# AegisIK/DistMLIP

Hardware: NVIDIA B200
Metric: atoms/sec (energy+forces) CHGNet a-Si r_cut=5A (higher is better)
Workload: dtype f32

## Files before the change

### distmlip_b200/csrc/kernels_tc.cu

```cuda
#include "kernels.cuh"
#include "tc_common.cuh"

namespace b2m {

static int l2pf_level() {
  static const int v = [] {
    const char* e = getenv("B2M_L2_PREFETCH");
    return e ? atoi(e) : 1;
  }();
  return v;
}


__global__ void k_edge_basis(int64_t E, const float4* __restrict__ e_vec, RadialParams rp, float* __restrict__ be,
                             float* __restrict__ dbe) {
  const int64_t i = blockIdx.x * (int64_t)blockDim.x + threadIdx.x;
  if (i >= E * 3) return;
  const int64_t e = i / 3;
  const int part = (int)(i % 3);
  const float d = e_vec[e].w;
  float b[4] = {0.f, 0.f, 0.f, 0.f}, db[4] = {0.f, 0.f, 0.f, 0.f};
  for (int j = 0; j < 4; j++) {
    const int k = part * 4 + j;
    if (k < 9) rbf_env_both(d, rp.freq[k], rp, b[j], db[j]);
// ... 476 lines not shown
          const float4 g4 = *reinterpret_cast<const float4*>(gmrow + c);
          const float uu[4] = {u4.x, u4.y, u4.z, u4.w}, vv[4] = {v4.x, v4.y, v4.z, v4.w}, gg[4] = {g4.x, g4.y, g4.z, g4.w};
          float wab4[4], wabp4[4];
          radial_dot4(wabW, c, bek, wab4);
          if (br == 0) radial_dot4(wabW, c, dbek, wabp4);
#pragma unroll
          for (int j = 0; j < 4; j++) {
            const float wab = wab4[j];
            const float su = sigm_(uu[j]), oG = sigm_(vv[j]);
            const float oL = uu[j] * su;
            float g;
            if (br == 0) {
              g = gg[j] * oG * wab * (su * (1.f + uu[j] * (1.f - su)));
              gdpart = fmaf(gg[j] * oL * oG, wabp4[j], gdpart);
            } else {
              g = gg[j] * oL * wab * oG * (1.f - oG);
            }
            if (!valid) g = 0.f;
            const uint32_t h = tf32_hi_bits(g);
            hi[4 * i + j] = h;
            lo[4 * i + j] = __float_as_uint(g - __uint_as_float(h));
          }
        }
        tmem_st16(tlane + COL_H + c0 + ch * 16, hi);
        tmem_st16(tlane + COL_H + 64 + c0 + ch * 16, lo);
      }
      tc_wait_st();
      tc_fence_before();
      __syncthreads();
      if (tid == 0) {
        tc_fence_after();
        uint32_t acc = 0;
#pragma unroll
        for (int term = 0; term < 3; term++) {
          const uint32_t acol = term == 1 ? 64u : 0u;
          const uint32_t bsel = w2t_addr + (uint32_t)(br * 2 + (term == 2 ? 1 : 0)) * 4096u * 4u;
#pragma unroll
          for (int ks = 0; ks < 8; ks++) {
            umma_ts(tbase + COL_D + br * 64, tbase + COL_H + acol + ks * 8, umma_desc(bsel + ks * 2048u, 1024u, 128u),
                    kIdescN64, acc);
            acc = 1;
          }
        }
        umma_commit(&mbar[br + 1]);
      }
      mbar_wait_(&mbar[br + 1], phase);
      tc_fence_after();
#pragma unroll
      for (int ch = 0; ch < NCH; ch++) {
        uint32_t v[16];
        tmem_ld16(tlane + COL_D + br * 64 + c0 + ch * 16, v);
        tc_wait_ld();
#pragma unroll
        for (int i = 0; i < 16; i++) ds[ch * 16 + i] *= __uint_as_float(v[i]);
      }
      if (!viaQ) {
#pragma unroll
        for (int i = 0; i < CPT; i++) {
          const float4* Mj = reinterpret_cast<const float4*>(Mrow + (cb + i) * 12);
#pragma unroll
          for (int k4 = 0; k4 < 3; k4++) {
            const float4 m = Mj[k4];
            ffma2(gbeM[4 * k4], gbeM[4 * k4 + 1], ds[i], m.x, m.y);
            ffma2(gbeM[4 * k4 + 2], gbeM[4 * k4 + 3], ds[i], m.z, m.w);
          }
        }
      }
      if (need_gx) {
#pragma unroll 1
        for (int hp = 0; hp < 2; hp++) {
          if ((q >> 1) == hp) {
            const int rr = r - hp * 64;
#pragma unroll
            for (int i = 0; i < CPT; i++) stage[rr * 65 + c0 + i] = ds[i];
          }
          __syncthreads();
          {
            constexpr int RPP = 64 / (NTHR / 16);
            const int c4 = tid & 15, part = tid >> 4;
            const int col = br * 64 + c4 * 4;
            float s0 = 0.f, s1 = 0.f, s2 = 0.f, s3 = 0.f;
            int cur = -1;
            const int rbeg = part * RPP;
            for (int rr = rbeg; rr < rbeg + RPP; rr++) {
              const int row = hp * 64 + rr;
              const int k = s_dst[row];
              const float v0 = stage[rr * 65 + c4 * 4], v1 = stage[rr * 65 + c4 * 4 + 1], v2 = stage[rr * 65 + c4 * 4 + 2],
                          v3 = stage[rr * 65 + c4 * 4 + 3];
              if (k != cur) {
                if (cur >= 0) red_add_v4(&a.gC[(size_t)cur * D2 + col], s0, s1, s2, s3);
                cur = k;
                s0 = s1 = s2 = s3 = 0.f;
              }
              if (k >= 0) {
                s0 += v0, s1 += v1, s2 += v2, s3 += v3;
                red_add_v4(&a.gA[(size_t)s_src[row] * D2 + col], v0, v1, v2, v3);
                const int bnd = s_bond[row];
                if (useQ && bnd >= 0) *reinterpret_cast<float4*>(&a.gQ[(size_t)bnd * D2 + col]) = make_float4(v0, v1, v2, v3);
              }
            }
            if (cur >= 0) red_add_v4(&a.gC[(size_t)cur * D2 + col], s0, s1, s2, s3);
          }
          __syncthreads();
        }
      }
    }
    phase ^= 1;
    {
      float s = gdpart;
#pragma unroll
      for (int k = 0; k < 9; k++) s = fmaf(gbeM[k], dbek[k], s);
      stage[tid] = valid ? s : 0.f;
      tc_fence_before();
      __syncthreads();
      if (tid < nvalid) {
        float tot = 0.f;
#pragma unroll
        for (int pp = 0; pp < NP; pp++) tot += stage[pp * 128 + tid];
        a.gd[e0 + tid] += tot;
      }
      __syncthreads();
    }
  }
  tc_fence_before();
  __syncthreads();
  if (warp == 0) asm volatile("tcgen05.dealloc.cta_group::1.sync.aligned.b32 %0, %1;" ::"r"(tbase), "r"(256u));
}

void launch_atomconv_bwd_tc(cudaStream_t st, const AtomConvArgs& a, const AtomConvTcW& w, int num_sms) {
  if (a.E <= 0) return;
  static PerDeviceOnce attr;
  if (auto once_ = attr.first(); once_) {
    B2M_CK(cudaFuncSetAttribute(k_atomconv_bwd_tc<256>, cudaFuncAttributeMaxDynamicSharedMemorySize, (int)BwdTcSmem::bytes));
    B2M_CK(cudaFuncSetAttribute(k_atomconv_bwd_tc<512>, cudaFuncAttributeMaxDynamicSharedMemorySize, (int)BwdTcSmem::bytes));
  }
  const int64_t ntiles = (a.E + 127) / 128;
  const int grid = (int)std::min<int64_t>(ntiles, 2 * (int64_t)num_sms);
  static const int nthr = [] {
    const char* v = getenv("B2M_BWD_THREADS");
    return (v && atoi(v) == 512) ? 512 : 256;
  }();
  AtomConvTcW wl = w;
  wl.l2pf = l2pf_level() >= 1;
  if (nthr == 512)
    k_atomconv_bwd_tc<512><<<grid, 512, BwdTcSmem::bytes, st>>>(a, wl);
  else
    k_atomconv_bwd_tc<256><<<grid, 256, BwdTcSmem::bytes, st>>>(a, wl);
  B2M_CK(cudaGetLastError());
  g_launch_count++;
}

constexpr bool kFwdPrefetchDefault = true;
void launch_atomconv_fwd_tc(cudaStream_t st, const AtomConvArgs& a, const AtomConvTcW& w, int num_sms) {
  if (a.E <= 0) return;
  static PerDeviceOnce attr;
  if (auto once_ = attr.first(); once_) {
    B2M_CK(cudaFuncSetAttribute(k_atomconv_fwd_tc<256, false>, cudaFuncAttributeMaxDynamicSharedMemorySize, (int)FwdTcSmem::bytes));
    B2M_CK(cudaFuncSetAttribute(k_atomconv_fwd_tc<256, true>, cudaFuncAttributeMaxDynamicSharedMemorySize, (int)FwdTcSmem::bytes));
    B2M_CK(cudaFuncSetAttribute(k_atomconv_fwd_tc<512, false>, cudaFuncAttributeMaxDynamicSharedMemorySize, (int)FwdTcSmem::bytes));
  }
  const int64_t ntiles = (a.E + 127) / 128;
  const int grid = (int)std::min<int64_t>(ntiles, 2 * (int64_t)num_sms);
  static const int nthr = [] {
    const char* v = getenv("B2M_FWD_THREADS");
    return (v && atoi(v) == 512) ? 512 : 256;
  }();
  static const bool pf = [] {
    const char* v = getenv("B2M_FWD_PREFETCH");
    return v ? atoi(v) != 0 : kFwdPrefetchDefault;
  }();
  AtomConvTcW wl = w;
  wl.l2pf = l2pf_level() >= 1;
  if (nthr == 512)
    k_atomconv_fwd_tc<512, false><<<grid, 512, FwdTcSmem::bytes, st>>>(a, wl);
  else if (pf)
    k_atomconv_fwd_tc<256, true><<<grid, 256, FwdTcSmem::bytes, st>>>(a, wl);
  else
    k_atomconv_fwd_tc<256, false><<<grid, 256, FwdTcSmem::bytes, st>>>(a, wl);
  B2M_CK(cudaGetLastError());
  g_launch_count++;
}

}

namespace b2m {


struct LineTcSmem {
  static constexpr int kBar = 0;
  static constexpr int kWA = 64;
  static constexpr int kWB = kWA + 16384;
  static constexpr int kB2 = kWB + 16384;
  static constexpr int kGrp = kB2 + 128;
  static constexpr int kGrpSize = 64 * 65 + 2 * 3 * 128;
  static constexpr int kTotal = kGrp + 2 * kGrpSize;
  static constexpr size_t bytes = (size_t)kTotal * 4;
};

template <bool HIDDEN>
__global__ void __launch_bounds__(512, 1) k_line_fwd_tc(const LineArgs a, const LineTcW w) {
  extern __shared__ __align__(1024) float smem[];
  const int tid = threadIdx.x;
  const int g = tid >> 8, gt = tid & 255;
  const int warp = gt >> 5, lane = tid & 31;
  const int q = warp & 3, half = warp >> 2;
  const int r = q * 32 + lane, c0 = half * 32;
  uint64_t* mbar = reinterpret_cast<uint64_t*>(smem + LineTcSmem::kBar) + g * 6;
  uint32_t* tptr = reinterpret_cast<uint32_t*>(smem + LineTcSmem::kBar + 48);
  float* WAs = smem + LineTcSmem::kWA;
  float* WBs = smem + LineTcSmem::kWB;
  float* b2s = smem + LineTcSmem::kB2;
  float* stage = smem + LineTcSmem::kGrp + g * LineTcSmem::kGrpSize;
  int* s_a = reinterpret_cast<int*>(stage + 64 * 65);
  int* s_b = s_a + 128;
  int* s_c = s_b + 128;

  if ((tid >> 5) == 0) {
    asm volatile("tcgen05.alloc.cta_group::1.sync.aligned.shared::cta.b32 [%0], %1;" ::"r"(s_u32(tptr)), "r"(512u));
    asm volatile("tcgen05.relinquish_alloc_permit.cta_group::1.sync.aligned;");
  }
  if (gt == 0) {
    for (int i = 0; i < 6; i++) mbar_init_(&mbar[i], 1);
    asm volatile("fence.mbarrier_init.release.cluster;" ::: "memory");
  }
  if (gt < 128) {
    const int64_t e = (2 * (int64_t)blockIdx.x + g) * 128 + gt;
    const bool ok = e < a.A;
    s_a[gt] = ok ? a.a_in[e] : 0, s_b[gt] = ok ? a.a_out[e] : -1, s_c[gt] = ok ? a.a_ctr[e] : 0;
  }
  for (int i = tid; i < 4096; i += 512) reinterpret_cast<float4*>(WAs)[i] = reinterpret_cast<const float4*>(w.Wgcan)[i];
  if (HIDDEN)
    for (int i = tid; i < 4096; i += 512) reinterpret_cast<float4*>(WBs)[i] = reinterpret_cast<const float4*>(w.W2can)[i];
  if (tid < 128) b2s[tid] = (HIDDEN && a.b2) ? a.b2[tid] : 0.f;
  asm volatile("fence.proxy.async.shared::cta;" ::: "memory");
  tc_fence_before();
  __syncthreads();
  tc_fence_after();
  const uint32_t tbase = *tptr + (uint32_t)g * 256u;
  const uint32_t tlane = tbase + ((uint32_t)(q * 32) << 16);
  constexpr uint32_t COL_H = 0, COL_D = 128;
  const uint32_t wa_addr = s_u32(WAs), wb_addr = s_u32(WBs);
  uint32_t phase = 0;

  const int64_t ntiles = (a.A + 127) / 128;
  const int64_t tstride = 2 * (int64_t)gridDim.x;
  int* idxb = s_a;
  int buf = 0;
  for (int64_t t = 2 * (int64_t)blockIdx.x + g; t < ntiles; t += tstride, buf ^= 1) {
    const int64_t r0 = t * 128;
    const int nvalid = (int)min((int64_t)128, a.A - r0);
    const int64_t tn = t + tstride;
    s_a = idxb + buf * 384, s_b = s_a + 128, s_c = s_a + 256;
    int nia = 0, nib = -1, nic = 0;
    if (tn < ntiles && gt < 128 && tn * 128 + gt < a.A) nia = a.a_in[tn * 128 + gt], nib = a.a_out[tn * 128 + gt], nic = a.a_ctr[tn * 128 + gt];
    if (tn < ntiles) {
      asm volatile("prefetch.global.L2 [%0];" ::"l"(reinterpret_cast<const char*>(a.ang + tn * (128 * 64)) + gt * 128));
    }
    const bool valid = r < nvalid;
    const int ia = s_a[r], ib = s_b[r], ic = s_c[r];
    const float4* ang4 = reinterpret_cast<const float4*>(a.ang);
    float angv[32];
    {
#pragma unroll
      for (int ch = 0; ch < 2; ch++) {
        uint32_t hi[16], lo[16];
#pragma unroll
        for (int i = 0; i < 4; i++) {
          float4 x = ang4[tl4<16>(t, r, c0 + ch * 16 + i * 4)];
          if (!valid) x = make_float4(0.f, 0.f, 0.f, 0.f);
          const float xv[4] = {x.x, x.y, x.z, x.w};
#pragma unroll
          for (int j = 0; j < 4; j++) {
            angv[ch * 16 + 4 * i + j] = xv[j];
            const uint32_t h = tf32_hi_bits(xv[j]);
            hi[4 * i + j] = h;
            lo[4 * i + j] = __float_as_uint(xv[j] - __uint_as_float(h));
          }
        }
        tmem_st16(tlane + COL_H + c0 + ch * 16, hi);
        tmem_st16(tlane + COL_H + 64 + c0 + ch * 16, lo);
      }
    }
    tc_wait_st();
    tc_fence_before();
    gbar(g);
    if (gt == 0) {
      tc_fence_after();
      uint32_t acc = 0;
#pragma unroll
      for (int term = 0; term < 3; term++) {
        const uint32_t acol = term == 1 ? 64u : 0u;
        const uint32_t bsel = wa_addr + (term == 2 ? 8192u * 4u : 0u);
#pragma unroll
        for (int ks = 0; ks < 8; ks++) {
          umma_ts(tbase + COL_D, tbase + COL_H + acol + ks * 8, umma_desc(bsel + ks * 4096u, 2048u, 128u), kIdescN128, acc);
          acc = 1;
        }
      }
      umma_commit(&mbar[0]);
    }
    const float* Harow = a.Ha + (size_t)ia * D2;
    const float* Hbrow = a.Hb + (size_t)(valid ? ib : 0) * D2;
    const float* Xcrow = a.Xc + (size_t)ic * D2;
    if (HIDDEN) {
#pragma unroll 1
      for (int br = 0; br < 2; br++) {
        mbar_wait_(&mbar[br], phase);
        tc_fence_after();
        const int cb = br * 64 + c0;
#pragma unroll
        for (int ch = 0; ch < 2; ch++) {
          uint32_t v[16], hi[16], lo[16];
          tmem_ld16(tlane + COL_D + cb + ch * 16, v);
          tc_wait_ld();
          float dsv[16];
#pragma unroll
          for (int i = 0; i < 4; i++) {
            const float4 x = *reinterpret_cast<const float4*>(Harow + cb + ch * 16 + i * 4);
            const float4 y = *reinterpret_cast<const float4*>(Hbrow + cb + ch * 16 + i * 4);
            const float4 z = *reinterpret_cast<const float4*>(Xcrow + cb + ch * 16 + i * 4);
            const float p4[4] = {__uint_as_float(v[4 * i]) + x.x + y.x + z.x, __uint_as_float(v[4 * i + 1]) + x.y + y.y + z.y,
                                 __uint_as_float(v[4 * i + 2]) + x.z + y.z + z.z,
                                 __uint_as_float(v[4 * i + 3]) + x.w + y.w + z.w};
#pragma unroll
            for (int j = 0; j < 4; j++) {
              const float sg = sigm_(p4[j]);
              const float hval = valid ? p4[j] * sg : 0.f;
              dsv[4 * i + j] = sg * (1.f + p4[j] * (1.f - sg));
              const uint32_t h = tf32_hi_bits(hval);
              hi[4 * i + j] = h;
              lo[4 * i + j] = __float_as_uint(hval - __uint_as_float(h));
            }
          }
          if (a.ds_save != nullptr && valid) {
            float4* pd = reinterpret_cast<float4*>(a.ds_save);
#pragma unroll
            for (int i = 0; i < 4; i++)
              __stcs(&pd[tl4<32>(t, r, cb + ch * 16 + 4 * i)], make_float4(dsv[4 * i], dsv[4 * i + 1], dsv[4 * i + 2], dsv[4 * i + 3]));
          }
          tmem_st16(tlane + COL_H + c0 + ch * 16, hi);
          tmem_st16(tlane + COL_H + 64 + c0 + ch * 16, lo);
        }
        tc_wait_st();
        tc_fence_before();
        gbar(g);
        if (gt == 0) {
          tc_fence_after();
          uint32_t acc = 0;
#pragma unroll
          for (int term = 0; term < 3; term++) {
            const uint32_t acol = term == 1 ? 64u : 0u;
            const uint32_t bsel = wb_addr + (uint32_t)(br * 2 + (term == 2 ? 1 : 0)) * 4096u * 4u;
#pragma unroll
            for (int ks = 0; ks < 8; ks++) {
              umma_ts(tbase + COL_D + br * 64, tbase + COL_H + acol + ks * 8, umma_desc(bsel + ks * 2048u, 1024u, 128u),
                      kIdescN64, acc);
              acc = 1;
            }
          }
          umma_commit(&mbar[br + 1]);
        }
      }
      mbar_wait_(&mbar[2], phase);
      tc_fence_after();
    } else {
      mbar_wait_(&mbar[0], phase);
      tc_fence_after();
    }
    float mv[32];
#pragma unroll
    for (int ch = 0; ch < 2; ch++) {
      uint32_t u[16], v[16];
      tmem_ld16(tlane + COL_D + c0 + ch * 16, u);
      tmem_ld16(tlane + COL_D + 64 + c0 + ch * 16, v);
      tc_wait_ld();
      float uf[16], vf[16];
      if (HIDDEN) {
#pragma unroll
        for (int i = 0; i < 16; i++) {
          uf[i] = __uint_as_float(u[i]) + b2s[c0 + ch * 16 + i];
          vf[i] = __uint_as_float(v[i]) + b2s[64 + c0 + ch * 16 + i];
        }
      } else {
#pragma unroll
        for (int i = 0; i < 4; i++) {
          const int cL = c0 + ch * 16 + i * 4, cG = 64 + cL;
          const float4 x = *reinterpret_cast<const float4*>(Harow + cL);
          const float4 y = *reinterpret_cast<const float4*>(Hbrow + cL);
          const float4 z = *reinterpret_cast<const float4*>(Xcrow + cL);
          const float4 x2 = *reinterpret_cast<const float4*>(Harow + cG);
          const float4 y2 = *reinterpret_cast<const float4*>(Hbrow + cG);
          const float4 z2 = *reinterpret_cast<const float4*>(Xcrow + cG);
          uf[4 * i] = __uint_as_float(u[4 * i]) + x.x + y.x + z.x;
          uf[4 * i + 1] = __uint_as_float(u[4 * i + 1]) + x.y + y.y + z.y;
          uf[4 * i + 2] = __uint_as_float(u[4 * i + 2]) + x.z + y.z + z.z;
          uf[4 * i + 3] = __uint_as_float(u[4 * i + 3]) + x.w + y.w + z.w;
          vf[4 * i] = __uint_as_float(v[4 * i]) + x2.x + y2.x + z2.x;
          vf[4 * i + 1] = __uint_as_float(v[4 * i + 1]) + x2.y + y2.y + z2.y;
          vf[4 * i + 2] = __uint_as_float(v[4 * i + 2]) + x2.z + y2.z + z2.z;
          vf[4 * i + 3] = __uint_as_float(v[4 * i + 3]) + x2.w + y2.w + z2.w;
        }
      }
      if (a.uv_save != nullptr && valid) {
        float4* puv = reinterpret_cast<float4*>(a.uv_save);
#pragma unroll
        for (int i = 0; i < 4; i++) {
          __stcs(&puv[tl4<32>(t, r, c0 + ch * 16 + 4 * i)], make_float4(uf[4 * i], uf[4 * i + 1], uf[4 * i + 2], uf[4 * i + 3]));
          __stcs(&puv[tl4<32>(t, r, 64 + c0 + ch * 16 + 4 * i)], make_float4(vf[4 * i], vf[4 * i + 1], vf[4 * i + 2], vf[4 * i + 3]));
        }
      }
#pragma unroll
      for (int i = 0; i < 16; i++) mv[ch * 16 + i] = valid ? silu_(uf[i]) * sigm_(vf[i]) : 0.f;
    }
    phase ^= 1;
    tc_fence_before();
    if (HIDDEN) {
#pragma unroll 1
      for (int hp = 0; hp < 2; hp++) {
        if ((q >> 1) == hp) {
          const int rr = r - hp * 64;
#pragma unroll
          for (int i = 0; i < 32; i++) stage[rr * 65 + c0 + i] = mv[i];
        }
        gbar(g);
        {
          const int c = gt & 63, part = gt >> 6;
          float sum = 0.f;
          int cur = -1;
          const int rbeg = part * 16;
          for (int rr = rbeg; rr < rbeg + 16; rr++) {
            const int k = s_b[hp * 64 + rr];
            if (k != cur) {
              if (cur >= 0) atomicAdd(&a.aggB[(size_t)cur * D + c], sum);
              cur = k;
              sum = 0.f;
            }
            if (k >= 0) sum += stage[rr * 65 + c];
          }
          if (cur >= 0) atomicAdd(&a.aggB[(size_t)cur * D + c], sum);
        }
        if (hp == 1 && gt < 128) {
          int* nb_ = idxb + (buf ^ 1) * 384;
          nb_[gt] = nia, nb_[128 + gt] = nib, nb_[256 + gt] = nic;
        }
        gbar(g);
      }
    } else {
      if (valid) {
        float4* po = reinterpret_cast<float4*>(a.ang_out);
#pragma unroll
        for (int i = 0; i < 8; i++)
          po[tl4<16>(t, r, c0 + 4 * i)] = make_float4(angv[4 * i] + mv[4 * i], angv[4 * i + 1] + mv[4 * i + 1], angv[4 * i + 2] + mv[4 * i + 2],
                              angv[4 * i + 3] + mv[4 * i + 3]);
      }
      if (gt < 128) {
        int* nb_ = idxb + (buf ^ 1) * 384;
        nb_[gt] = nia, nb_[128 + gt] = nib, nb_[256 + gt] = nic;
      }
      gbar(g);
    }
  }
  tc_fence_before();
  __syncthreads();
  if ((tid >> 5) == 0) asm volatile("tcgen05.dealloc.cta_group::1.sync.aligned.b32 %0, %1;" ::"r"(*tptr), "r"(512u));
}

template <bool HIDDEN>
__global__ void __launch_bounds__(512, 1) k_line_bwd_tc(const LineArgs a, const LineTcW w) {
  extern __shared__ __align__(1024) float smem[];
  const int tid = threadIdx.x;
  const int g = tid >> 8, gt = tid & 255;
  const int warp = gt >> 5, lane = tid & 31;
  const int q = warp & 3, half = warp >> 2;
  const int r = q * 32 + lane, c0 = half * 32;
  uint64_t* mbar = reinterpret_cast<uint64_t*>(smem + LineTcSmem::kBar) + g * 6;
  uint32_t* tptr = reinterpret_cast<uint32_t*>(smem + LineTcSmem::kBar + 48);
  float* WAs = smem + LineTcSmem::kWA;
  float* WBs = smem + LineTcSmem::kWB;
  float* stage = smem + LineTcSmem::kGrp + g * LineTcSmem::kGrpSize;
  int* s_a = reinterpret_cast<int*>(stage + 64 * 65);
  int* s_b = s_a + 128;
  int* s_c = s_b + 128;

  if ((tid >> 5) == 0) {
    asm volatile("tcgen05.alloc.cta_group::1.sync.aligned.shared::cta.b32 [%0], %1;" ::"r"(s_u32(tptr)), "r"(512u));
    asm volatile("tcgen05.relinquish_alloc_permit.cta_group::1.sync.aligned;");
  }
  if (gt == 0) {
    for (int i = 0; i < 6; i++) mbar_init_(&mbar[i], 1);
    asm volatile("fence.mbarrier_init.release.cluster;" ::: "memory");
  }
  if (gt < 128) {
    const int64_t e = (2 * (int64_t)blockIdx.x + g) * 128 + gt;
    const bool ok = e < a.A;
    s_a[gt] = ok ? a.a_in[e] : -1, s_b[gt] = ok ? a.a_out[e] : -1, s_c[gt] = ok ? a.a_ctr[e] : -1;
  }
  for (int i = tid; i < 4096; i += 512) reinterpret_cast<float4*>(WAs)[i] = reinterpret_cast<const float4*>(w.WgTcan)[i];
  if (HIDDEN)
    for (int i = tid; i < 4096; i += 512) reinterpret_cast<float4*>(WBs)[i] = reinterpret_cast<const float4*>(w.W2Tcan)[i];
  asm volatile("fence.proxy.async.shared::cta;" ::: "memory");
  tc_fence_before();
  __syncthreads();
  tc_fence_after();
  const uint32_t tbase = *tptr + (uint32_t)g * 256u;
  const uint32_t tlane = tbase + ((uint32_t)(q * 32) << 16);
  constexpr uint32_t COL_H = 0, COL_D = 128, COL_G = 192;
  const uint32_t wa_addr = s_u32(WAs), wb_addr = s_u32(WBs);
  uint32_t phase = 0;

  const int64_t ntiles = (a.A + 127) / 128;
  const int64_t tstride = 2 * (int64_t)gridDim.x;
  int* idxb = s_a;
  int buf = 0;
  for (int64_t t = 2 * (int64_t)blockIdx.x + g; t < ntiles; t += tstride, buf ^= 1) {
    const int64_t r0 = t * 128;
    const int nvalid = (int)min((int64_t)128, a.A - r0);
    const int64_t tn = t + tstride;
    s_a = idxb + buf * 384, s_b = s_a + 128, s_c = s_a + 256;
    int nia = -1, nib = -1, nic = -1;
    if (tn < ntiles && gt < 128 && tn * 128 + gt < a.A) nia = a.a_in[tn * 128 + gt], nib = a.a_out[tn * 128 + gt], nic = a.a_ctr[tn * 128 + gt];
    if (tn < ntiles) {
      asm volatile("prefetch.global.L2 [%0];" ::"l"(reinterpret_cast<const char*>(a.gang + tn * (128 * 64)) + gt * 128));
      if (w.l2pf) {
        l2_prefetch(a.uv + tn * (128 * 128), 128 * 128 * 4, gt, 256);
        if (HIDDEN) l2_prefetch(a.ds + tn * (128 * 128), 128 * 128 * 4, gt, 256);
      }
    }
    const bool valid = r < nvalid;
    const int ib = s_b[r];
    const float4* uv4 = reinterpret_cast<const float4*>(a.uv);
    const float* gmrow = a.gaggB + (size_t)(valid && HIDDEN ? ib : 0) * D;
    const float4* gang4 = reinterpret_cast<const float4*>(a.gang);
#pragma unroll 1
    for (int br = 0; br < 2; br++) {
      float gp[32];
      const int cb = br * 64 + c0;
      if (br == 1) {
        mbar_wait_(&mbar[2], phase);
        tc_fence_after();
      }
#pragma unroll
      for (int ch = 0; ch < 2; ch++) {
        uint32_t hi[16], lo[16];
#pragma unroll
        for (int i = 0; i < 4; i++) {
          const int c = c0 + ch * 16 + i * 4;
          const float4 u4 = uv4[tl4<32>(t, r, c)];
          const float4 v4 = uv4[tl4<32>(t, r, 64 + c)];
          const float4 g4 = HIDDEN ? *reinterpret_cast<const float4*>(gmrow + c) : gang4[tl4<16>(t, r, c)];
          const float uu[4] = {u4.x, u4.y, u4.z, u4.w}, vv[4] = {v4.x, v4.y, v4.z, v4.w}, gg[4] = {g4.x, g4.y, g4.z, g4.w};
#pragma unroll
          for (int j = 0; j < 4; j++) {
            const float su = sigm_(uu[j]), oG = sigm_(vv[j]);
            float gval;
            if (br == 0)
              gval = gg[j] * oG * (su * (1.f + uu[j] * (1.f - su)));
            else
              gval = gg[j] * (uu[j] * su) * oG * (1.f - oG);
            if (!valid) gval = 0.f;
            gp[ch * 16 + 4 * i + j] = gval;
            const uint32_t h = tf32_hi_bits(gval);
            hi[4 * i + j] = h;
            lo[4 * i + j] = __float_as_uint(gval - __uint_as_float(h));
          }
        }
        if (HIDDEN) {
          tmem_st16(tlane + COL_H + c0 + ch * 16, hi);
          tmem_st16(tlane + COL_H + 64 + c0 + ch * 16, lo);
        }
      }
      if (HIDDEN) {
        tc_wait_st();
        tc_fence_before();
        gbar(g);
        if (gt == 0) {
          tc_fence_after();
          uint32_t acc = 0;
#pragma unroll
          for (int term = 0; term < 3; term++) {
            const uint32_t acol = term == 1 ? 64u : 0u;
            const uint32_t bsel = wb_addr + (uint32_t)(br * 2 + (term == 2 ? 1 : 0)) * 4096u * 4u;
#pragma unroll
            for (int ks = 0; ks < 8; ks++) {
              umma_ts(tbase + COL_D, tbase + COL_H + acol + ks * 8, umma_desc(bsel + ks * 2048u, 1024u, 128u), kIdescN64, acc);
              acc = 1;
            }
          }
          umma_commit(&mbar[br]);
        }
        const float4* ds4 = reinterpret_cast<const float4*>(a.ds);
        float4 dsr[8];
#pragma unroll
        for (int i = 0; i < 8; i++) dsr[i] = __ldcs(ds4 + tl4<32>(t, r, cb + i * 4));
        mbar_wait_(&mbar[br], phase);
        tc_fence_after();
#pragma unroll
        for (int ch = 0; ch < 2; ch++) {
          uint32_t v[16];
          tmem_ld16(tlane + COL_D + c0 + ch * 16, v);
          tc_wait_ld();
#pragma unroll
          for (int i = 0; i < 4; i++) {
            const float4 d4 = dsr[ch * 4 + i];
            gp[ch * 16 + 4 * i] = __uint_as_float(v[4 * i]) * d4.x;
            gp[ch * 16 + 4 * i + 1] = __uint_as_float(v[4 * i + 1]) * d4.y;
            gp[ch * 16 + 4 * i + 2] = __uint_as_float(v[4 * i + 2]) * d4.z;
            gp[ch * 16 + 4 * i + 3] = __uint_as_float(v[4 * i + 3]) * d4.w;
          }
        }
      }
#pragma unroll
      for (int ch = 0; ch < 2; ch++) {
        uint32_t hi[16], lo[16];
#pragma unroll
        for (int i = 0; i < 16; i++) {
          const float x = valid ? gp[ch * 16 + i] : 0.f;
          const uint32_t h = tf32_hi_bits(x);
          hi[i] = h;
          lo[i] = __float_as_uint(x - __uint_as_float(h));
        }
        tmem_st16(tlane + COL_H + c0 + ch * 16, hi);
        tmem_st16(tlane + COL_H + 64 + c0 + ch * 16, lo);
      }
      tc_wait_st();
      tc_fence_before();
      gbar(g);
      if (gt == 0) {
        tc_fence_after();
        uint32_t acc = br == 0 ? 0u : 1u;
#pragma unroll
        for (int term = 0; term < 3; term++) {
          const uint32_t acol = term == 1 ? 64u : 0u;
          const uint32_t bsel = wa_addr + (uint32_t)(br * 2 + (term == 2 ? 1 : 0)) * 4096u * 4u;
#pragma unroll
          for (int ks = 0; ks < 8; ks++) {
            umma_ts(tbase + COL_G, tbase + COL_H + acol + ks * 8, umma_desc(bsel + ks * 2048u, 1024u, 128u), kIdescN64, acc);
            acc = 1;
          }
        }
        umma_commit(&mbar[2 + br]);
      }
#pragma unroll 1
      for (int hp = 0; hp < 2; hp++) {
        if ((q >> 1) == hp) {
          const int rr = r - hp * 64;
#pragma unroll
          for (int i = 0; i < 32; i++) stage[rr * 65 + c0 + i] = gp[i];
        }
        gbar(g);
        {
          const int c4 = gt & 15, part = gt >> 4;
          const int col = br * 64 + c4 * 4;
          float sb0 = 0.f, sb1 = 0.f, sb2 = 0.f, sb3 = 0.f, sc0 = 0.f, sc1 = 0.f, sc2 = 0.f, sc3 = 0.f;
          int curb = -1, curc = -1;
          const int rbeg = part * 4;
          for (int rr = rbeg; rr < rbeg + 4; rr++) {
            const int rowi = hp * 64 + rr;
            const int kb = s_b[rowi], kc = s_c[rowi];
            const float v0 = stage[rr * 65 + c4 * 4], v1 = stage[rr * 65 + c4 * 4 + 1], v2 = stage[rr * 65 + c4 * 4 + 2],
                        v3 = stage[rr * 65 + c4 * 4 + 3];
            if (kb != curb) {
              if (curb >= 0) red_add_v4(&a.gHb[(size_t)curb * D2 + col], sb0, sb1, sb2, sb3);
              curb = kb;
              sb0 = sb1 = sb2 = sb3 = 0.f;
            }
            if (kc != curc) {
              if (curc >= 0) red_add_v4(&a.gXc[(size_t)curc * D2 + col], sc0, sc1, sc2, sc3);
              curc = kc;
              sc0 = sc1 = sc2 = sc3 = 0.f;
            }
            if (kb >= 0) {
              sb0 += v0, sb1 += v1, sb2 += v2, sb3 += v3;
              sc0 += v0, sc1 += v1, sc2 += v2, sc3 += v3;
              red_add_v4(&a.gHa[(size_t)s_a[rowi] * D2 + col], v0, v1, v2, v3);
            }
          }
          if (curb >= 0) red_add_v4(&a.gHb[(size_t)curb * D2 + col], sb0, sb1, sb2, sb3);
          if (curc >= 0) red_add_v4(&a.gXc[(size_t)curc * D2 + col], sc0, sc1, sc2, sc3);
        }
        gbar(g);
      }
    }
    {
      float4* pg = reinterpret_cast<float4*>(a.gang);
      float4 o[8];
#pragma unroll
      for (int i = 0; i < 8; i++) o[i] = valid ? pg[tl4<16>(t, r, c0 + 4 * i)] : make_float4(0.f, 0.f, 0.f, 0.f);
      mbar_wait_(&mbar[3], phase);
      tc_fence_after();
#pragma unroll
      for (int ch = 0; ch < 2; ch++) {
        uint32_t v[16];
        tmem_ld16(tlane + COL_G + c0 + ch * 16, v);
        tc_wait_ld();
        if (valid) {
#pragma unroll
          for (int i = 0; i < 4; i++) {
            float4 x = o[ch * 4 + i];
            x.x += __uint_as_float(v[4 * i]), x.y += __uint_as_float(v[4 * i + 1]);
            x.z += __uint_as_float(v[4 * i + 2]), x.w += __uint_as_float(v[4 * i + 3]);
            pg[tl4<16>(t, r, c0 + ch * 16 + 4 * i)] = x;
          }
        }
      }
    }
    phase ^= 1;
    if (gt < 128) {
      int* nb_ = idxb + (buf ^ 1) * 384;
      nb_[gt] = nia, nb_[128 + gt] = nib, nb_[256 + gt] = nic;
    }
    tc_fence_before();
    gbar(g);
  }
  tc_fence_before();
  __syncthreads();
  if ((tid >> 5) == 0) asm volatile("tcgen05.dealloc.cta_group::1.sync.aligned.b32 %0, %1;" ::"r"(*tptr), "r"(512u));
}

void launch_line_fwd_tc(cudaStream_t st, const LineArgs& a, const LineTcW& w, bool hidden, int num_sms) {
  if (a.A <= 0) return;
  static PerDeviceOnce attr;
  if (auto once_ = attr.first(); once_) {
    B2M_CK(cudaFuncSetAttribute(k_line_fwd_tc<true>, cudaFuncAttributeMaxDynamicSharedMemorySize, (int)LineTcSmem::bytes));
    B2M_CK(cudaFuncSetAttribute(k_line_fwd_tc<false>, cudaFuncAttributeMaxDynamicSharedMemorySize, (int)LineTcSmem::bytes));
  }
  const int64_t ntiles = (a.A + 127) / 128;
  const int grid = (int)std::min<int64_t>((ntiles + 1) / 2, (int64_t)num_sms);
  LineTcW wl = w;
  wl.l2pf = l2pf_level() >= 2;
  if (hidden)
    k_line_fwd_tc<true><<<grid, 512, LineTcSmem::bytes, st>>>(a, wl);
  else
    k_line_fwd_tc<false><<<grid, 512, LineTcSmem::bytes, st>>>(a, wl);
  B2M_CK(cudaGetLastError());
  g_launch_count++;
}
void launch_line_bwd_tc(cudaStream_t st, const LineArgs& a, const LineTcW& w, bool hidden, int num_sms) {
  if (a.A <= 0) return;
  static PerDeviceOnce attr;
  if (auto once_ = attr.first(); once_) {
    B2M_CK(cudaFuncSetAttribute(k_line_bwd_tc<true>, cudaFuncAttributeMaxDynamicSharedMemorySize, (int)LineTcSmem::bytes));
    B2M_CK(cudaFuncSetAttribute(k_line_bwd_tc<false>, cudaFuncAttributeMaxDynamicSharedMemorySize, (int)LineTcSmem::bytes));
// ... 385 lines not shown
```

### distmlip_b200/csrc/tc_common.cuh

```cuda
#pragma once
#include "kernels.cuh"

namespace b2m {

__device__ __forceinline__ float sigm_(float x) {
  float e, r;
  asm("ex2.approx.ftz.f32 %0, %1;" : "=f"(e) : "f"(x * -1.4426950408889634f));
  asm("rcp.approx.ftz.f32 %0, %1;" : "=f"(r) : "f"(1.f + e));
  return r;
}
__device__ __forceinline__ float silu_(float x) { return x * sigm_(x); }
__device__ __forceinline__ float dsilu_(float x) {
  const float sg = sigm_(x);
  return sg * (1.f + x * (1.f - sg));
}
__device__ __forceinline__ uint32_t s_u32(const void* p) { return (uint32_t)__cvta_generic_to_shared(p); }

__device__ __forceinline__ uint32_t tf32_hi_bits(float x) {
  uint32_t u;
  asm("cvt.rna.tf32.f32 %0, %1;" : "=r"(u) : "f"(x));
  return u;
}
__device__ __forceinline__ uint64_t umma_desc(uint32_t saddr, uint32_t lbo, uint32_t sbo) {
  return (uint64_t)((saddr & 0x3FFFF) >> 4) | ((uint64_t)(lbo >> 4) << 16) | ((uint64_t)(sbo >> 4) << 32) | (1ull << 46);
}
__device__ __forceinline__ void umma_ts(uint32_t d_tmem, uint32_t a_tmem, uint64_t bdesc, uint32_t idesc, uint32_t acc) {
  asm volatile(
      "{\n\t.reg .pred p;\n\tsetp.ne.b32 p, %4, 0;\n\t"
      "tcgen05.mma.cta_group::1.kind::tf32 [%0], [%1], %2, %3, p;\n\t}" ::"r"(d_tmem),
      "r"(a_tmem), "l"(bdesc), "r"(idesc), "r"(acc)
      : "memory");
}
__device__ __forceinline__ void umma_commit(uint64_t* bar) {
  asm volatile("tcgen05.commit.cta_group::1.mbarrier::arrive::one.shared::cluster.b64 [%0];" ::"r"(s_u32(bar)) : "memory");
}
__device__ __forceinline__ void tc_fence_before() { asm volatile("tcgen05.fence::before_thread_sync;" ::: "memory"); }
__device__ __forceinline__ void tc_fence_after() { asm volatile("tcgen05.fence::after_thread_sync;" ::: "memory"); }
__device__ __forceinline__ void tc_wait_st() { asm volatile("tcgen05.wait::st.sync.aligned;" ::: "memory"); }
__device__ __forceinline__ void tc_wait_ld() { asm volatile("tcgen05.wait::ld.sync.aligned;" ::: "memory"); }
__device__ __forceinline__ void tmem_st16(uint32_t addr, const uint32_t (&v)[16]) {
  asm volatile(
      "tcgen05.st.sync.aligned.32x32b.x16.b32 [%0], {%1, %2, %3, %4, %5, %6, %7, %8, %9, %10, %11, %12, %13, %14, %15, %16};" ::
          "r"(addr),
      "r"(v[0]), "r"(v[1]), "r"(v[2]), "r"(v[3]), "r"(v[4]), "r"(v[5]), "r"(v[6]), "r"(v[7]), "r"(v[8]), "r"(v[9]),
      "r"(v[10]), "r"(v[11]), "r"(v[12]), "r"(v[13]), "r"(v[14]), "r"(v[15])
      : "memory");
}
__device__ __forceinline__ void tmem_ld16(uint32_t addr, uint32_t (&v)[16]) {
  asm volatile(
      "tcgen05.ld.sync.aligned.32x32b.x16.b32 {%0, %1, %2, %3, %4, %5, %6, %7, %8, %9, %10, %11, %12, %13, %14, %15}, [%16];"
      : "=r"(v[0]), "=r"(v[1]), "=r"(v[2]), "=r"(v[3]), "=r"(v[4]), "=r"(v[5]), "=r"(v[6]), "=r"(v[7]), "=r"(v[8]),
        "=r"(v[9]), "=r"(v[10]), "=r"(v[11]), "=r"(v[12]), "=r"(v[13]), "=r"(v[14]), "=r"(v[15])
      : "r"(addr)
      : "memory");
}
__device__ __forceinline__ void mbar_init_(uint64_t* bar, uint32_t count) {
  asm volatile("mbarrier.init.shared::cta.b64 [%0], %1;" ::"r"(s_u32(bar)), "r"(count) : "memory");
}
__device__ __forceinline__ void mbar_wait_(uint64_t* bar, uint32_t parity) {
  uint32_t ok = 0;
  const uint32_t addr = s_u32(bar);
  do {
    asm volatile(
        "{\n\t.reg .pred p;\n\tmbarrier.try_wait.parity.shared::cta.b64 p, [%1], %2;\n\tselp.u32 %0, 1, 0, p;\n\t}"
        : "=r"(ok)
        : "r"(addr), "r"(parity)
        : "memory");
  } while (!ok);
}
__device__ __forceinline__ void gbar(int g) { asm volatile("bar.sync %0, 256;" ::"r"(g + 1) : "memory"); }
__device__ __forceinline__ float ipow_(float x, int n) {
  float r = 1.f;
  for (int i = 0; i < n; i++) r *= x;
  return r;
}
__device__ __forceinline__ float rbf_env_val(float d, float freq, const RadialParams& rp) {
  const float invd = 1.f / d;
  float s, c;
  sincosf(d * (freq / rp.rc), &s, &c);
  const float rbf = rp.norm * s * invd;
  const int p = rp.p;
  const float c1 = -(p + 1) * (p + 2) * 0.5f, c2 = (float)(p * (p + 2)), c3 = -p * (p + 1) * 0.5f;
  const float rho = rbf / rp.rc;
  const float r0 = ipow_(rho, p), r1 = r0 * rho, r2 = r1 * rho;
  const float env = 1.f + c1 * r0 + c2 * r1 + c3 * r2;
  return rbf <= rp.rc ? env * rbf : 0.f;
}

template <int NC4>
__device__ __forceinline__ size_t tl4(int64_t tile, int r, int c) {
  return ((size_t)(tile * NC4 + (c >> 2)) * 128 + r);
}

__device__ __forceinline__ void red_add_v4(float* addr, float a, float b, float c, float d) {
  asm volatile("red.global.add.v4.f32 [%0], {%1, %2, %3, %4};" ::"l"(addr), "f"(a), "f"(b), "f"(c), "f"(d) : "memory");
}

__device__ __forceinline__ void l2_prefetch(const void* base, int bytes, int tid, int nthr) {
  const char* p = reinterpret_cast<const char*>(base);
  for (int o = tid * 128; o < bytes; o += nthr * 128) asm volatile("prefetch.global.L2 [%0];" ::"l"(p + o));
}

__device__ __forceinline__ void ffma2(float& d0, float& d1, float a, float b0, float b1) {
  uint64_t A, B, C, D;
  asm("mov.b64 %0, {%1, %2};" : "=l"(A) : "f"(a), "f"(a));
  asm("mov.b64 %0, {%1, %2};" : "=l"(B) : "f"(b0), "f"(b1));
  asm("mov.b64 %0, {%1, %2};" : "=l"(C) : "f"(d0), "f"(d1));
  asm("fma.rn.f32x2 %0, %1, %2, %3;" : "=l"(D) : "l"(A), "l"(B), "l"(C));
  asm("mov.b64 {%0, %1}, %2;" : "=f"(d0), "=f"(d1) : "l"(D));
}
__device__ __forceinline__ void radial_dot16(const float* WT, int col0, const float (&b)[9], float (&w)[16]) {
#pragma unroll
  for (int i = 0; i < 16; i++) w[i] = 0.f;
#pragma unroll
  for (int k = 0; k < 9; k++) {
#pragma unroll
    for (int c4 = 0; c4 < 4; c4++) {
      const float4 x = *reinterpret_cast<const float4*>(WT + k * 64 + col0 + c4 * 4);
      ffma2(w[4 * c4], w[4 * c4 + 1], b[k], x.x, x.y);
      ffma2(w[4 * c4 + 2], w[4 * c4 + 3], b[k], x.z, x.w);
    }
  }
}

__device__ __forceinline__ void radial_dot4(const float* WT, int col0, const float (&b)[9], float (&w)[4]) {
  w[0] = w[1] = w[2] = w[3] = 0.f;
#pragma unroll
  for (int k = 0; k < 9; k++) {
    const float4 x = *reinterpret_cast<const float4*>(WT + k * 64 + col0);
    ffma2(w[0], w[1], b[k], x.x, x.y);
    ffma2(w[2], w[3], b[k], x.z, x.w);
  }
}

constexpr uint32_t kIdescN64 = (1u << 4) | (2u << 7) | (2u << 10) | (8u << 17) | (8u << 24);
constexpr uint32_t kIdescN128 = (1u << 4) | (2u << 7) | (2u << 10) | (16u << 17) | (8u << 24);

__device__ __forceinline__ void rbf_env_both(float d, float freq, const RadialParams& rp, float& be, float& dbe) {
  const float invd = 1.f / d;
  const float wq = freq / rp.rc;
  float s, c;
  sincosf(d * wq, &s, &c);
  const float rbf = rp.norm * s * invd;
  const float drbf = rp.norm * (wq * c * invd - s * invd * invd);
  const int p = rp.p;
  const float c1 = -(p + 1) * (p + 2) * 0.5f, c2 = (float)(p * (p + 2)), c3 = -p * (p + 1) * 0.5f;
  const float rho = rbf / rp.rc;
  const float rm1 = ipow_(rho, p - 1);
  const float r0 = rm1 * rho, r1 = r0 * rho, r2 = r1 * rho;
  const float env = 1.f + c1 * r0 + c2 * r1 + c3 * r2;
  const float denv = (c1 * p * rm1 + c2 * (p + 1) * r0 + c3 * (p + 2) * r1) / rp.rc;
  const bool ok = rbf <= rp.rc;
  be = ok ? env * rbf : 0.f;
  dbe = ok ? (env + rbf * denv) * drbf : 0.f;
}

__device__ __forceinline__ void mbar_expect_tx_(uint64_t* bar, uint32_t bytes) {
  asm volatile("mbarrier.arrive.expect_tx.shared::cta.b64 _, [%0], %1;" ::"r"(s_u32(bar)), "r"(bytes) : "memory");
}
__device__ __forceinline__ void bulk_g2s_(void* dst_smem, const void* src_gmem, uint32_t bytes, uint64_t* bar) {
  asm volatile("cp.async.bulk.shared::cluster.global.mbarrier::complete_tx::bytes [%0], [%1], %2, [%3];" ::"r"(
                   s_u32(dst_smem)),
               "l"(src_gmem), "r"(bytes), "r"(s_u32(bar))
               : "memory");
}


__device__ __forceinline__ void tmem_st8(uint32_t addr, const uint32_t (&v)[8]) {
  asm volatile("tcgen05.st.sync.aligned.32x32b.x8.b32 [%0], {%1, %2, %3, %4, %5, %6, %7, %8};" ::"r"(addr), "r"(v[0]),
               "r"(v[1]), "r"(v[2]), "r"(v[3]), "r"(v[4]), "r"(v[5]), "r"(v[6]), "r"(v[7])
               : "memory");
}
__device__ __forceinline__ void tmem_ld8(uint32_t addr, uint32_t (&v)[8]) {
  asm volatile("tcgen05.ld.sync.aligned.32x32b.x8.b32 {%0, %1, %2, %3, %4, %5, %6, %7}, [%8];"
               : "=r"(v[0]), "=r"(v[1]), "=r"(v[2]), "=r"(v[3]), "=r"(v[4]), "=r"(v[5]), "=r"(v[6]), "=r"(v[7])
               : "r"(addr)
               : "memory");
}
__device__ __forceinline__ void cp_async16_(void* dst_smem, const void* src_gmem) {
  asm volatile("cp.async.cg.shared.global [%0], [%1], 16;" ::"r"(s_u32(dst_smem)), "l"(src_gmem) : "memory");
}
__device__ __forceinline__ void cp_async_arrive_(uint64_t* bar) {
  asm volatile("cp.async.mbarrier.arrive.noinc.shared::cta.b64 [%0];" ::"r"(s_u32(bar)) : "memory");
}

__device__ __forceinline__ uint64_t pk2(float a, float b) {
  uint64_t r;
  asm("mov.b64 %0, {%1, %2};" : "=l"(r) : "f"(a), "f"(b));
  return r;
}
__device__ __forceinline__ void upk2(uint64_t v, float& a, float& b) { asm("mov.b64 {%0, %1}, %2;" : "=f"(a), "=f"(b) : "l"(v)); }
__device__ __forceinline__ uint64_t add2(uint64_t a, uint64_t b) {
  uint64_t r;
  asm("add.rn.f32x2 %0, %1, %2;" : "=l"(r) : "l"(a), "l"(b));
  return r;
}
__device__ __forceinline__ uint64_t sub2(uint64_t a, uint64_t b) {
  uint64_t r;
  asm("sub.rn.f32x2 %0, %1, %2;" : "=l"(r) : "l"(a), "l"(b));
  return r;
}
__device__ __forceinline__ uint64_t mul2(uint64_t a, uint64_t b) {
  uint64_t r;
  asm("mul.rn.f32x2 %0, %1, %2;" : "=l"(r) : "l"(a), "l"(b));
  return r;
}
__device__ __forceinline__ uint64_t fma2(uint64_t a, uint64_t b, uint64_t c) {
  uint64_t r;
  asm("fma.rn.f32x2 %0, %1, %2, %3;" : "=l"(r) : "l"(a), "l"(b), "l"(c));
  return r;
}
__device__ __forceinline__ float ex2_(float x) {
  float e;
  asm("ex2.approx.ftz.f32 %0, %1;" : "=f"(e) : "f"(x));
  return e;
}
__device__ __forceinline__ float rcp_(float x) {
  float r;
  asm("rcp.approx.ftz.f32 %0, %1;" : "=f"(r) : "f"(x));
  return r;
}
}
```

Before: 5.030 million.

## Prefetch next gather rows via bulk L2 prefetch, hoist row sums, vectorize scatter

Issues cp.async.bulk L2 prefetches for the next tile's Ha/Hb/Xc rows. The three-way gather sum is moved ahead of the mbarrier wait, so global loads overlap the tensor-core MMA. The segmented scatter-add now has each thread accumulate 4 columns over 4 rows and emit red.global.add.v4 instead of scalar atomicAdd, which cuts the number of atomic operations. The trade-offs are more register pressure from the early-loaded sums and shorter per-thread segments, which can mean more atomics when neighbours repeat. A profiling script is also added.

```diff
diff --git a/distmlip_b200/csrc/kernels_tc.cu b/distmlip_b200/csrc/kernels_tc.cu
--- a/distmlip_b200/csrc/kernels_tc.cu
+++ b/distmlip_b200/csrc/kernels_tc.cu
@@ -802,12 +802,23 @@
     const float* Harow = a.Ha + (size_t)ia * D2;
     const float* Hbrow = a.Hb + (size_t)(valid ? ib : 0) * D2;
     const float* Xcrow = a.Xc + (size_t)ic * D2;
+    auto prefetch_next_rows = [&] {
+      if (gt < 128 && nib >= 0) {
+        l2_prefetch_bulk(a.Ha + (size_t)nia * D2, D2 * 4);
+        l2_prefetch_bulk(a.Hb + (size_t)nib * D2, D2 * 4);
+        l2_prefetch_bulk(a.Xc + (size_t)nic * D2, D2 * 4);
+      }
+    };
+    float gsu[16];
     if (HIDDEN) {
+      prefetch_next_rows();
 #pragma unroll 1
       for (int br = 0; br < 2; br++) {
+        const int cb = br * 64 + c0;
+        float gs[32];
+        sum3_row(Harow + cb, Hbrow + cb, Xcrow + cb, gs);
         mbar_wait_(&mbar[br], phase);
         tc_fence_after();
-        const int cb = br * 64 + c0;
 #pragma unroll
         for (int ch = 0; ch < 2; ch++) {
           uint32_t v[16], hi[16], lo[16];
@@ -816,12 +827,9 @@
           float dsv[16];
 #pragma unroll
           for (int i = 0; i < 4; i++) {
-            const float4 x = *reinterpret_cast<const float4*>(Harow + cb + ch * 16 + i * 4);
-            const float4 y = *reinterpret_cast<const float4*>(Hbrow + cb + ch * 16 + i * 4);
-            const float4 z = *reinterpret_cast<const float4*>(Xcrow + cb + ch * 16 + i * 4);
-            const float p4[4] = {__uint_as_float(v[4 * i]) + x.x + y.x + z.x, __uint_as_float(v[4 * i + 1]) + x.y + y.y + z.y,
-                                 __uint_as_float(v[4 * i + 2]) + x.z + y.z + z.z,
-                                 __uint_as_float(v[4 * i + 3]) + x.w + y.w + z.w};
+            const float* s = gs + ch * 16 + i * 4;
+            const float p4[4] = {__uint_as_float(v[4 * i]) + s[0], __uint_as_float(v[4 * i + 1]) + s[1],
+                                 __uint_as_float(v[4 * i + 2]) + s[2], __uint_as_float(v[4 * i + 3]) + s[3]};
 #pragma unroll
             for (int j = 0; j < 4; j++) {
               const float sg = sigm_(p4[j]);
@@ -864,8 +872,10 @@
       mbar_wait_(&mbar[2], phase);
       tc_fence_after();
     } else {
+      sum3_row(Harow + c0, Hbrow + c0, Xcrow + c0, gsu);
       mbar_wait_(&mbar[0], phase);
       tc_fence_after();
+      prefetch_next_rows();
     }
     float mv[32];
 #pragma unroll
@@ -882,23 +892,18 @@
           vf[i] = __uint_as_float(v[i]) + b2s[64 + c0 + ch * 16 + i];
         }
       } else {
-#pragma unroll
-        for (int i = 0; i < 4; i++) {
-          const int cL = c0 + ch * 16 + i * 4, cG = 64 + cL;
-          const float4 x = *reinterpret_cast<const float4*>(Harow + cL);
-          const float4 y = *reinterpret_cast<const float4*>(Hbrow + cL);
-          const float4 z = *reinterpret_cast<const float4*>(Xcrow + cL);
-          const float4 x2 = *reinterpret_cast<const float4*>(Harow + cG);
-          const float4 y2 = *reinterpret_cast<const float4*>(Hbrow + cG);
-          const float4 z2 = *reinterpret_cast<const float4*>(Xcrow + cG);
-          uf[4 * i] = __uint_as_float(u[4 * i]) + x.x + y.x + z.x;
-          uf[4 * i + 1] = __uint_as_float(u[4 * i + 1]) + x.y + y.y + z.y;
-          uf[4 * i + 2] = __uint_as_float(u[4 * i + 2]) + x.z + y.z + z.z;
-          uf[4 * i + 3] = __uint_as_float(u[4 * i + 3]) + x.w + y.w + z.w;
-          vf[4 * i] = __uint_as_float(v[4 * i]) + x2.x + y2.x + z2.x;
-          vf[4 * i + 1] = __uint_as_float(v[4 * i + 1]) + x2.y + y2.y + z2.y;
-          vf[4 * i + 2] = __uint_as_float(v[4 * i + 2]) + x2.z + y2.z + z2.z;
-          vf[4 * i + 3] = __uint_as_float(v[4 * i + 3]) + x2.w + y2.w + z2.w;
+        float gu[16], gv[16];
+        if (ch == 0) {
+#pragma unroll
+          for (int i = 0; i < 16; i++) gu[i] = gsu[i];
+        } else {
+          sum3_row(Harow + c0 + 16, Hbrow + c0 + 16, Xcrow + c0 + 16, gu);
+        }
+        sum3_row(Harow + 64 + c0 + ch * 16, Hbrow + 64 + c0 + ch * 16, Xcrow + 64 + c0 + ch * 16, gv);
+#pragma unroll
+        for (int i = 0; i < 16; i++) {
+          uf[i] = __uint_as_float(u[i]) + gu[i];
+          vf[i] = __uint_as_float(v[i]) + gv[i];
         }
       }
       if (a.uv_save != nullptr && valid) {
@@ -924,20 +929,23 @@
         }
         gbar(g);
         {
-          const int c = gt & 63, part = gt >> 6;
-          float sum = 0.f;
+          const int c4 = (gt & 15) * 4, part = gt >> 4;
+          float s0 = 0.f, s1 = 0.f, s2 = 0.f, s3 = 0.f;
           int cur = -1;
-          const int rbeg = part * 16;
-          for (int rr = rbeg; rr < rbeg + 16; rr++) {
+          const int rbeg = part * 4;
+          for (int rr = rbeg; rr < rbeg + 4; rr++) {
             const int k = s_b[hp * 64 + rr];
             if (k != cur) {
-              if (cur >= 0) atomicAdd(&a.aggB[(size_t)cur * D + c], sum);
+              if (cur >= 0) red_add_v4(&a.aggB[(size_t)cur * D + c4], s0, s1, s2, s3);
               cur = k;
-              sum = 0.f;
+              s0 = s1 = s2 = s3 = 0.f;
             }
-            if (k >= 0) sum += stage[rr * 65 + c];
-          }
-          if (cur >= 0) atomicAdd(&a.aggB[(size_t)cur * D + c], sum);
+            if (k >= 0) {
+              const float* st4 = stage + rr * 65 + c4;
+              s0 += st4[0], s1 += st4[1], s2 += st4[2], s3 += st4[3];
+            }
+          }
+          if (cur >= 0) red_add_v4(&a.aggB[(size_t)cur * D + c4], s0, s1, s2, s3);
         }
         if (hp == 1 && gt < 128) {
           int* nb_ = idxb + (buf ^ 1) * 384;
diff --git a/distmlip_b200/csrc/tc_common.cuh b/distmlip_b200/csrc/tc_common.cuh
--- a/distmlip_b200/csrc/tc_common.cuh
+++ b/distmlip_b200/csrc/tc_common.cuh
@@ -99,6 +99,21 @@
 __device__ __forceinline__ void l2_prefetch(const void* base, int bytes, int tid, int nthr) {
   const char* p = reinterpret_cast<const char*>(base);
   for (int o = tid * 128; o < bytes; o += nthr * 128) asm volatile("prefetch.global.L2 [%0];" ::"l"(p + o));
+}
+
+__device__ __forceinline__ void l2_prefetch_bulk(const void* p, uint32_t bytes) {
+  asm volatile("cp.async.bulk.prefetch.L2.global [%0], %1;" ::"l"(p), "r"(bytes));
+}
+template <int N>
+__device__ __forceinline__ void sum3_row(const float* x, const float* y, const float* z, float (&s)[N]) {
+#pragma unroll
+  for (int i = 0; i < N / 4; i++) {
+    const float4 a = *reinterpret_cast<const float4*>(x + 4 * i);
+    const float4 b = *reinterpret_cast<const float4*>(y + 4 * i);
+    const float4 c = *reinterpret_cast<const float4*>(z + 4 * i);
+    s[4 * i] = a.x + b.x + c.x, s[4 * i + 1] = a.y + b.y + c.y;
+    s[4 * i + 2] = a.z + b.z + c.z, s[4 * i + 3] = a.w + b.w + c.w;
+  }
 }
 
 __device__ __forceinline__ void ffma2(float& d0, float& d1, float a, float b0, float b1) {
diff --git a/profiles/r03_kernel_times.py b/profiles/r03_kernel_times.py
--- /dev/null
+++ b/profiles/r03_kernel_times.py
@@ -0,0 +1,29 @@
+import csv
+import os
+import runpy
+import sys
+
+import torch
+from torch.profiler import ProfilerActivity, profile
+
+out, bench_args = sys.argv[1], sys.argv[2:]
+sys.argv = ["bench.py"] + bench_args
+sys.path.insert(0, os.getcwd())
+with profile(activities=[ProfilerActivity.CUDA]) as prof:
+    try:
+        runpy.run_path("bench.py", run_name="__main__")
+    except SystemExit:
+        pass
+    torch.cuda.synchronize()
+rows = {}
+for ev in prof.events():
+    if ev.device_type == torch.autograd.DeviceType.CUDA and "k_line_" in ev.name:
+        n, t = rows.get(ev.name, (0, 0.0))
+        rows[ev.name] = (n + 1, t + ev.device_time)
+with open(out, "w", newline="") as f:
+    w = csv.writer(f)
+    w.writerow(["kernel", "launches", "total_us", "mean_us"])
+    for k, (n, t) in sorted(rows.items()):
+        w.writerow([k, n, round(t, 1), round(t / n, 1)])
+for k, (n, t) in sorted(rows.items()):
+    print(f"{k:45s} {n:5d} {t / n:9.1f} us", file=sys.stderr)
```

New measurement: 5.036 million, median of 6. No clear change (+0.1%).
